# VikParuchuri/surya

Hardware: AMD Instinct MI355X
Metric: text-lines/sec recognised (whole node) (higher is better)
Workload: dtype bf16; 1 GPU; RecognitionPredictor device loop, 256 ragged 64x{128..512} crops/GPU, batch 256, max_tokens=48, REC-FULL synthetic weights (conditioned recipe, seed 0), tiles resident in HBM; parallelism=1 GPU, weights=conditioned

## Files before the change

### surya_amd/csrc/attn_mfma.h

```cpp
#pragma once
#include "common.h"
#include "kernels.h"

namespace sa {

typedef short s16x4 __attribute__((ext_vector_type(4)));

template <typename T, int D>
__global__ __launch_bounds__(128) void attn_mfma_kernel(const T* __restrict__ q, const T* __restrict__ k,
                                                        const T* __restrict__ v, T* __restrict__ out, AttnSegs sg,
                                                        long q_row, long q_head, long k_row, long k_head, long o_row, long o_head,
                                                        int group, int causal, float scale) {
    static_assert(D % 16 == 0 && D <= 128, "head dim");
    static_assert(sizeof(T) == 2, "16-bit storage types");
    constexpr int KC = 64;
    constexpr int PK = D + 8;
    constexpr int NKK = D / 16;
    constexpr int NDB = (D + 31) / 32;
    constexpr int CPR = D / 8;
    __shared__ __attribute__((aligned(16))) T ks[(KC + 1) * PK];
    __shared__ __attribute__((aligned(16))) T vs[(KC + 1) * PK];

    const int tile = blockIdx.x, head = blockIdx.y, kvh = head / group;
    const int seg = sg.tile_seg[tile], q0 = sg.tile_q0[tile], L = sg.seg_len[seg];
    const int tid = threadIdx.x, lane = tid & 63, wave = tid >> 6;
    const int ql = lane & 31, h = lane >> 5;
    const int qi = q0 + wave * 32 + ql;

    u32x4 qf[NKK];
    {
        const T* qp = q + sg.q_off[seg] + (long)min(qi, L - 1) * q_row + (long)head * q_head + h * 8;
#pragma unroll
        for (int kk = 0; kk < NKK; ++kk) qf[kk] = *reinterpret_cast<const u32x4*>(qp + kk * 16);
    }
    f32x16 oacc[NDB];
#pragma unroll
    for (int db = 0; db < NDB; ++db)
#pragma unroll
        for (int r = 0; r < 16; ++r) oacc[db][r] = 0.f;
    float mrun = -INFINITY, lrun = 0.f;
    const float sl2 = scale * 1.44269504088896340736f;

    const int kend = causal ? min(L, q0 + 64) : L;
    const T* kbase = k + sg.k_off[seg] + (long)kvh * k_head;
    const T* vbase = v + sg.v_off[seg] + (long)kvh * k_head;
    const int tr_off = ((lane & 15) >> 2) * PK + ((lane >> 4) & 1) * 16 + (lane & 3) * 4 + h * 4 * PK;

    constexpr int NST = KC * CPR / 128;
    static_assert(KC * CPR % 128 == 0, "staging split");
    u32x4 kreg[NST], vreg[NST];
    auto fetch = [&](int kc) {
        const int nk = min(KC, kend - kc);
#pragma unroll
        for (int it = 0; it < NST; ++it) {
            const int c = tid + it * 128, r = min(c / CPR, nk - 1), cc = c % CPR;
            kreg[it] = *reinterpret_cast<const u32x4*>(kbase + (long)(kc + r) * k_row + cc * 8);
            vreg[it] = *reinterpret_cast<const u32x4*>(vbase + (long)(kc + r) * k_row + cc * 8);
        }
    };
    if (kend > 0) fetch(0);
    for (int kc = 0; kc < kend; kc += KC) {
        const int nk = min(KC, kend - kc);
#pragma unroll
        for (int it = 0; it < NST; ++it) {
            const int c = tid + it * 128, r = c / CPR, cc = c % CPR;
            const bool in = r < nk;
            const u32x4 z = {0u, 0u, 0u, 0u};
            *reinterpret_cast<u32x4*>(ks + r * PK + cc * 8) = in ? kreg[it] : z;
            *reinterpret_cast<u32x4*>(vs + r * PK + cc * 8) = in ? vreg[it] : z;
        }
        __syncthreads();
        if (kc + KC < kend) fetch(kc + KC);

        f32x16 sacc[2];
#pragma unroll
        for (int kb = 0; kb < 2; ++kb) {
#pragma unroll
            for (int r = 0; r < 16; ++r) sacc[kb][r] = 0.f;
            const T* kp = ks + (kb * 32 + ql) * PK + h * 8;
#pragma unroll
            for (int kk = 0; kk < NKK; ++kk) {
                const u32x4 kf = *reinterpret_cast<const u32x4*>(kp + kk * 16);
                sacc[kb] = H16<T>::mfma(kf, qf[kk], sacc[kb]);
            }
        }
        float bm = -INFINITY;
#pragma unroll
        for (int kb = 0; kb < 2; ++kb)
#pragma unroll
            for (int g = 0; g < 4; ++g)
#pragma unroll
                for (int r = 0; r < 4; ++r) {
                    const int j = kb * 32 + g * 8 + h * 4 + r;
                    const bool ok = (j < nk) && (!causal || (kc + j) <= qi);
                    const float sv = ok ? sacc[kb][4 * g + r] : -INFINITY;
                    sacc[kb][4 * g + r] = sv;
                    bm = fmaxf(bm, sv);
                }
        bm = fmaxf(bm, __shfl_xor(bm, 32, 64));
        const float mnew = fmaxf(mrun, bm);
        const float alpha = exp2f((mrun - mnew) * sl2);
        mrun = mnew;
        float psum = 0.f;
#pragma unroll
        for (int kb = 0; kb < 2; ++kb)
#pragma unroll
            for (int r = 0; r < 16; ++r) {
                const float pv = exp2f((sacc[kb][r] - mnew) * sl2);
                sacc[kb][r] = pv;
                psum += pv;
            }
        lrun = lrun * alpha + psum;
#pragma unroll
        for (int db = 0; db < NDB; ++db)
#pragma unroll
            for (int r = 0; r < 16; ++r) oacc[db][r] *= alpha;

#pragma unroll
        for (int t = 0; t < 4; ++t) {
            const int kb = t >> 1, o8 = (t & 1) * 8;
            u32x4 pf;
            pf[0] = H16<T>::pk(sacc[kb][o8 + 0], sacc[kb][o8 + 1]);
            pf[1] = H16<T>::pk(sacc[kb][o8 + 2], sacc[kb][o8 + 3]);
            pf[2] = H16<T>::pk(sacc[kb][o8 + 4], sacc[kb][o8 + 5]);
            pf[3] = H16<T>::pk(sacc[kb][o8 + 6], sacc[kb][o8 + 7]);
#pragma unroll
            for (int db = 0; db < NDB; ++db) {
                const T* vp = vs + t * 16 * PK + db * 32 + tr_off;
                const s16x4 lo = __builtin_amdgcn_ds_read_tr16_b64_v4i16((__attribute__((address_space(3))) s16x4*)(vp));
                const s16x4 hi = __builtin_amdgcn_ds_read_tr16_b64_v4i16((__attribute__((address_space(3))) s16x4*)(vp + 8 * PK));
                typedef short s16x8 __attribute__((ext_vector_type(8)));
                const s16x8 vf = __builtin_shufflevector(lo, hi, 0, 1, 2, 3, 4, 5, 6, 7);
                oacc[db] = H16<T>::mfma(vf, pf, oacc[db]);
            }
        }
        __syncthreads();
    }

    const float ltot = lrun + __shfl_xor(lrun, 32, 64);
    if (qi < L) {
        const float inv = 1.0f / ltot;
        T* op = out + sg.o_off[seg] + (long)qi * o_row + (long)head * o_head;
#pragma unroll
        for (int db = 0; db < NDB; ++db)
#pragma unroll
            for (int g = 0; g < 4; ++g) {
                const int d0 = db * 32 + g * 8 + h * 4;
                if (d0 < D) store4(op + d0, oacc[db][4 * g] * inv, oacc[db][4 * g + 1] * inv, oacc[db][4 * g + 2] * inv,
                                   oacc[db][4 * g + 3] * inv);
            }
    }
}

template <typename T>
int launch_attn(int D, const T* q, const T* k, const T* v, T* o, const AttnSegs& sg, int n_tiles, int heads, long q_row, long q_head,
                long k_row, long k_head, long o_row, long o_head, int group, int causal, float scale, hipStream_t s) {
    if (n_tiles <= 0) return SA_OK;
    auto go = [&](auto kern, int threads) {
        hipLaunchKernelGGL(kern, dim3(n_tiles, heads), dim3(threads), 0, s, q, k, v, o, sg, q_row, q_head, k_row, k_head, o_row, o_head, group,
                           causal, scale);
        return (int)hipGetLastError();
    };
    if constexpr (sizeof(T) == 2) {
        if (D == 32) return go(attn_mfma_kernel<T, 32>, 128);
        if (D == 64) return go(attn_mfma_kernel<T, 64>, 128);
        if (D == 80) return go(attn_mfma_kernel<T, 80>, 128);
        if (D == 128) return go(attn_mfma_kernel<T, 128>, 128);
    } else {
        static_assert(std::is_same<T, float>::value, "the VALU kernel is the fp32 reference-mode path only");
        if (D == 32) return go(attn_valu_kernel<T, 32>, 256);
        if (D == 64) return go(attn_valu_kernel<T, 64>, 256);
        if (D == 80) return go(attn_valu_kernel<T, 80>, 256);
        if (D == 128) return go(attn_valu_kernel<T, 128>, 256);
    }
    return SA_ERR_UNSUPPORTED;
}

}
```

### surya_amd/csrc/common.h

```cpp
#pragma once
#include <hip/hip_runtime.h>
#include <cstdlib>
#include <stdint.h>
#include <stdio.h>
#include <type_traits>

#include "../../include/surya_amd.h"

namespace sa {

typedef unsigned short bf16_t;
typedef __attribute__((ext_vector_type(4))) float f32x4;
typedef __attribute__((ext_vector_type(16))) float f32x16;
typedef __attribute__((ext_vector_type(8))) __bf16 bf16x8;
typedef unsigned int u32x4 __attribute__((ext_vector_type(4)));


#define SA_HIP(expr)                                                                                   \
    do {                                                                                               \
        hipError_t _e = (expr);                                                                        \
        if (_e != hipSuccess) {                                                                        \
            fprintf(stderr, "[surya_amd] %s:%d %s -> %s\n", __FILE__, __LINE__, #expr, hipGetErrorString(_e)); \
            return (int)_e;                                                                            \
        }                                                                                              \
// ... 214 lines not shown
__device__ __forceinline__ float hardswish_f(float x) {
    float t;
    asm("v_fma_f32 %0, %1, %2, 0.5 clamp" : "=v"(t) : "v"(x), "s"(1.0f / 6.0f));
    return x * t;
}
typedef float f32x2_hs __attribute__((ext_vector_type(2)));
__device__ __forceinline__ f32x2_hs hardswish_pk(f32x2_hs x) {
    f32x2_hs t;
    const f32x2_hs c = {1.0f / 6.0f, 1.0f / 6.0f};
    asm("v_pk_fma_f32 %0, %1, %2, 0.5 op_sel_hi:[1,0,0] clamp" : "=v"(t) : "v"(x), "s"(c));
    return x * t;
}

struct Tuning {
    int graph = 0;
    int split_target = 256;
    int split_min_kt = 4;
    int split_max = 8;
    int bigtile = 3;
    int bigtile_any = 0;
    int big_m_split = -1;
    int big_m_gateup = -1;
    int mx_big_m_split = -1;
    int mx_big_m_gateup = -1;
    int gateup_ring = 2;
    int dring = 1;
    int dring_min_kt = 0;
    int conv_persist = 3;
    int dwconv_pipe = 2;
    int conv_lean = 1;
    int bigtile_ratio_pct = 0;
    int bigtile_min_k = 0;
    int glds = 2;
    int dattn = 4;
    int rnorm = 2;
    int ghead = 2;
    int fuse_embed = 1;
    int kvprefetch = 0;
    int lmhead = 1;
    int dattn_db = 0;
    int lay_ln = 1;
    int det_head_blk = 1;
    int det_fuse = 1023;
    int det_up4 = 1;
    int fmb_chunk = 64;
    int persist = 1;
    int ocrerr_cls_only = 1;
};
inline Tuning& tuning() { static Tuning t; return t; }
inline int& tuning_epoch() { static int e = 0; return e; }

inline void poison_arena(void* p, size_t bytes) {
    static const bool on = [] { const char* e = getenv("SURYA_AMD_POISON"); return e && e[0] == '1'; }();
    if (on) { (void)hipMemset(p, 0xFF, bytes); (void)hipDeviceSynchronize(); }
}

struct AttrOnce {
    size_t granted[64] = {};
    template <typename F> void ensure(F kern, size_t lds) {
        int dev = 0;
        (void)hipGetDevice(&dev);
        size_t& g = granted[dev & 63];
        if (lds > g || g == 0) {
            (void)hipFuncSetAttribute(reinterpret_cast<const void*>(kern), hipFuncAttributeMaxDynamicSharedMemorySize, (int)lds);
            g = lds > g ? lds : g;
            if (g == 0) g = 1;
        }
    }
};

constexpr int SA_ALT_NONE = 0x7fffffff;
__device__ __forceinline__ bool alt_after(float v, int c, float pv, int pc) { return (v < pv) | ((v == pv) & (c > pc)); }
__device__ __forceinline__ bool alt_before(float v, int c, float bv, int bc) { return (v > bv) | ((v == bv) & (c < bc)); }
__device__ __forceinline__ float2 alt_next(const float2* cand, int n, float pv, int pc) {
    float cb = -INFINITY;
    int ci = SA_ALT_NONE;
    for (int k = 0; k < n; ++k) {
        const float v = cand[k].x;
        const int cc = __float_as_int(cand[k].y);
// ... 12 lines not shown
```

### surya_amd/csrc/decode_attn.h

```cpp
#pragma once
#include "gemm.h"

namespace sa {

#ifdef SA_DA_TIMING
__device__ unsigned long long sa_da_stamps[16];
#define SA_DA_STAMP(i) if (blockIdx.x == 64 && blockIdx.y == 0 && threadIdx.x == 0) sa_da_stamps[i] = wall_clock64();
#else
#define SA_DA_STAMP(i)
#endif

template <typename T, int D, int MAXG>
__global__ __launch_bounds__(256) void decode_attn_mfma_kernel(const float* __restrict__ qkv_part, int S, const T* __restrict__ qkv_bias,
                                                               T* __restrict__ out, T* __restrict__ kc, T* __restrict__ vc,
                                                               const int* __restrict__ active_slots, const int* __restrict__ row_len,
                                                               const float2* __restrict__ rope_cs, int nq, int nkv, int Tmax,
                                                               float scale) {
    constexpr int V16 = Ty<T>::V16;
    constexpr int CPRk = D / V16;
    constexpr int ROWB = D * (int)sizeof(T);
    constexpr int KT = (ROWB >= 512) ? 64 : 128;
    constexpr int XM = CPRk >= 16 ? 15 : CPRk - 1;
    constexpr int NCH = KT * CPRk / 256;
    static_assert(KT * CPRk % 256 == 0 && NCH >= 1 && D % 32 == 0 && MAXG <= 32, "geometry");
// ... 407 lines not shown
    }
    __syncthreads();
    SA_DA_STAMP(6)
    if (tid < G * (D / 4)) {
        const int oh = tid / (D / 4), od = (tid % (D / 4)) * 4;
        float mx = -INFINITY;
#pragma unroll
        for (int w = 0; w < 4; ++w) mx = fmaxf(mx, comb[(w * MAXG + oh) * CW + D]);
        float num[4] = {0.f, 0.f, 0.f, 0.f}, den = 0.f;
#pragma unroll
        for (int w = 0; w < 4; ++w) {
            const float* rec = comb + (w * MAXG + oh) * CW;
            const float e = (rec[D] == -INFINITY) ? 0.f : __expf(rec[D] - mx);
            const float4 o4 = *reinterpret_cast<const float4*>(rec + od);
            num[0] += e * o4.x; num[1] += e * o4.y; num[2] += e * o4.z; num[3] += e * o4.w;
            den += e * rec[D + 1];
        }
        const float inv = 1.0f / den;
        const long o_off = (long)a * nq * D + (long)(kvh * G + oh) * D + od;
        store4(out + o_off, num[0] * inv, num[1] * inv, num[2] * inv, num[3] * inv);
        if (out8) {
            const float q[4] = {Ty<T>::rnd(num[0] * inv), Ty<T>::rnd(num[1] * inv), Ty<T>::rnd(num[2] * inv), Ty<T>::rnd(num[3] * inv)};
            int e8;
            const uint32_t pk = mx_quant4_oct(q, e8);
            *reinterpret_cast<uint32_t*>(out8 + o_off) = pk;
            const int col = (kvh * G + oh) * D + od;
            if ((tid & 7) == 0) sout[((long)(col >> 7) * srows + a) * 4 + ((col >> 5) & 3)] = (uint8_t)e8;
        }
    }
    SA_DA_STAMP(7)
    SA_DA_STAMP(8)
}

template <int D, int MAXG, bool DB = false, typename T = bf16_t>
__global__ __launch_bounds__(256) void decode_attn_flash2_kernel(const float* __restrict__ qkv_part, int S, const T* __restrict__ qkv_bias,
                                                                 T* __restrict__ out, T* __restrict__ kc, T* __restrict__ vc,
                                                                 const int* __restrict__ active_slots, const int* __restrict__ row_len,
                                                                 const float2* __restrict__ rope_cs, int nq, int nkv, int Tmax,
                                                                 float scale, uint8_t* __restrict__ out8 = nullptr,
                                                                 uint8_t* __restrict__ sout = nullptr, int srows = 0) {
    static_assert(sizeof(T) == 2, "a 16-bit storage type");
    constexpr int CPR = D / 8;
    constexpr int ROWB = D * 2;
    constexpr int KT = 128;
    constexpr int RPI = 1024 / ROWB;
    constexpr int XM = CPR >= 16 ? 15 : CPR - 1;
    constexpr int NKK = D / 16, NDB = (D + 31) / 32;
    constexpr int CW = D + 4;
    constexpr int IPH = D / 8;
    static_assert(D % 32 == 0 && D <= 128 && MAXG <= 32 && 1024 % ROWB == 0, "geometry");
    static_assert((MAXG + 2) * IPH <= 256 && MAXG * CW * 4 <= 32 * ROWB, "one prologue pass; a wave's records fit its own K rows");
    extern __shared__ __attribute__((aligned(16))) unsigned char smem[];
    constexpr int NBUF = DB ? 2 : 1;
    constexpr int BUFB = 2 * KT * ROWB;
    unsigned char* Ks = smem;
    unsigned char* Vs = Ks + KT * ROWB;
    unsigned char* qT = smem + NBUF * BUFB;

    SA_DA_STAMP(0)
    const int G = nq / nkv;
    const int a = blockIdx.x, kvh = blockIdx.y;
    const int slot = active_slots[a];
    const int len = row_len[a];
    const int tid = threadIdx.x, lane = tid & 63, wave = tid >> 6;
    const int total = len + 1;
    const unsigned char* kb = reinterpret_cast<const unsigned char*>(kc + ((long)slot * nkv + kvh) * Tmax * D);
    const unsigned char* vb = reinterpret_cast<const unsigned char*>(vc + ((long)slot * nkv + kvh) * Tmax * D);
    typedef const __attribute__((address_space(1))) void* gptr_t;
    typedef __attribute__((address_space(3))) void* lptr_t;

    auto issue_tile = [&](int base, int buf) {
        const int rows = min(KT, (total - base + 15) & ~15);
        const int ngroups = (rows + RPI - 1) / RPI;
        unsigned char* Kd = Ks + buf * BUFB;
        unsigned char* Vd = Vs + buf * BUFB;
        for (int g = wave; g < ngroups; g += 4) {
            const int r = g * RPI + lane / CPR, pc = lane % CPR;
            const long j = min(base + r, max(len - 1, 0));
            if (base + r != len) {
                __builtin_amdgcn_global_load_lds((gptr_t)(kb + j * ROWB + ((pc ^ (r & XM)) << 4)), (lptr_t)(Kd + g * 1024), 16, 0, 0);
                __builtin_amdgcn_global_load_lds((gptr_t)(vb + j * ROWB + (pc << 4)), (lptr_t)(Vd + g * 1024), 16, 0, 0);
            }
        }
    };
    issue_tile(0, 0);
    SA_DA_STAMP(1)

    const int qkv_dim = (nq + 2 * nkv) * D;
    const int Mrows = gridDim.x;
    constexpr int half = D / 2;
    const int n_items = (G + 2) * IPH;
    const int item = min(tid, n_items - 1);
    const bool on = tid < n_items;
    const int hh = item / IPH, i0 = (item % IPH) * 4;
    const int col = (hh < G ? (kvh * G + hh) * D : (hh == G ? (nq + kvh) * D : (nq + nkv + kvh) * D)) + i0;
    const float* prow = qkv_part + (long)a * qkv_dim + col;
    const long sstride = (long)Mrows * qkv_dim;
    f32x4 plo[8], phi[8];
    const int SL = S <= 2 ? 2 : (S <= 4 ? 4 : 8);
    if (SL == 2) {
#pragma unroll
        for (int s = 0; s < 2; ++s) {
            plo[s] = *reinterpret_cast<const f32x4*>(prow + min(s, S - 1) * sstride);
            phi[s] = *reinterpret_cast<const f32x4*>(prow + min(s, S - 1) * sstride + half);
        }
#pragma unroll
        for (int s = 2; s < 8; ++s) { plo[s] = f32x4{0.f, 0.f, 0.f, 0.f}; phi[s] = plo[s]; }
    } else if (SL == 4) {
#pragma unroll
        for (int s = 0; s < 4; ++s) {
            plo[s] = *reinterpret_cast<const f32x4*>(prow + min(s, S - 1) * sstride);
            phi[s] = *reinterpret_cast<const f32x4*>(prow + min(s, S - 1) * sstride + half);
        }
#pragma unroll
        for (int s = 4; s < 8; ++s) { plo[s] = f32x4{0.f, 0.f, 0.f, 0.f}; phi[s] = plo[s]; }
    } else {
#pragma unroll
        for (int s = 0; s < 8; ++s) {
            plo[s] = *reinterpret_cast<const f32x4*>(prow + min(s, S - 1) * sstride);
            phi[s] = *reinterpret_cast<const f32x4*>(prow + min(s, S - 1) * sstride + half);
        }
    }
    float blo[4], bhi[4];
    load4(qkv_bias + col, blo);
    load4(qkv_bias + col + half, bhi);
    const float4 csA = *reinterpret_cast<const float4*>(rope_cs + (long)len * half + i0);
    const float4 csB = *reinterpret_cast<const float4*>(rope_cs + (long)len * half + i0 + 2);
    for (int i = tid; i < (32 - G) * CPR; i += 256)
        *reinterpret_cast<u32x4*>(qT + G * ROWB + i * 16) = u32x4{0u, 0u, 0u, 0u};
    SA_DA_STAMP(2)
    float xlo[4], xhi[4];
#pragma unroll
    for (int e = 0; e < 4; ++e) {
        float vl = blo[e], vh = bhi[e];
#pragma unroll
        for (int s = 0; s < 8; ++s) {
            const bool use = s < S;
            vl += use ? plo[s][e] : 0.f;
            vh += use ? phi[s][e] : 0.f;
        }
        xlo[e] = Ty<T>::rnd(vl); xhi[e] = Ty<T>::rnd(vh);
    }
    const float csn[4] = {csA.x, csA.z, csB.x, csB.z}, snn[4] = {csA.y, csA.w, csB.y, csB.w};
    float ylo[4], yhi[4];
#pragma unroll
    for (int e = 0; e < 4; ++e) {
        const float r1 = Ty<T>::rnd(__fmaf_rn(xlo[e], csn[e], -__fmul_rn(xhi[e], snn[e])));
        const float r2 = Ty<T>::rnd(__fmaf_rn(xhi[e], csn[e], __fmul_rn(xlo[e], snn[e])));
        ylo[e] = hh <= G ? r1 : xlo[e];
        yhi[e] = hh <= G ? r2 : xhi[e];
    }
    const int new_tile = len / KT, new_row = len % KT;
    auto lds_put4 = [&](unsigned char* rowp, int swz, int e0, const float (&v)[4], float mul) {
        const int c = e0 / 8, w = e0 % 8;
        store4(reinterpret_cast<T*>(rowp + ((c ^ swz) << 4)) + w, v[0] * mul, v[1] * mul, v[2] * mul, v[3] * mul);
    };
    auto put_new_rows = [&](int buf) {
        if (on && hh == G) {
            lds_put4(Ks + buf * BUFB + new_row * ROWB, new_row & XM, i0, ylo, 1.f);
            lds_put4(Ks + buf * BUFB + new_row * ROWB, new_row & XM, i0 + half, yhi, 1.f);
        } else if (on && hh == G + 1) {
            lds_put4(Vs + buf * BUFB + new_row * ROWB, 0, i0, ylo, 1.f);
            lds_put4(Vs + buf * BUFB + new_row * ROWB, 0, i0 + half, yhi, 1.f);
        }
    };
    if (on && hh < G) {
        lds_put4(qT + hh * ROWB, hh & XM, i0, ylo, scale);
        lds_put4(qT + hh * ROWB, hh & XM, i0 + half, yhi, scale);
    }
    if (new_tile == 0) put_new_rows(0);
    SA_DA_STAMP(3)
    asm volatile("s_waitcnt vmcnt(0)" ::: "memory");
    __syncthreads();
    if (on && hh >= G) {
        T* dst = (hh == G ? kc : vc) + (((long)slot * nkv + kvh) * Tmax + len) * D;
// ... 152 lines not shown
static inline size_t decode_attn_mfma_lds() {
    constexpr int ROWB = D * (int)sizeof(T);
    constexpr int KT = (ROWB >= 512) ? 64 : 128;
    return (size_t)2 * KT * ROWB + 32 * ROWB + (size_t)MAXG * KT * 4 + (size_t)(MAXG + 2) * D * 4 + 3 * MAXG * 4 + 64;
}

template <typename T>
struct DecodeAttnArgs {
    const float* qkv_part; int S;
    const T* qkv_bias;
    T* out;
    T *kcache, *vcache;
    const int *active_slots, *row_len;
    const float2* rope_cs;
    int rows, nq, nkv, d, max_kv_len;
    float scale;
    int ctx_bound = 0;
    uint8_t *out8 = nullptr, *sout = nullptr; int srows = 0;
};
template <typename T>
int launch_decode_attn(const DecodeAttnArgs<T>& a, hipStream_t s);
template <> int launch_decode_attn<fp16_t>(const DecodeAttnArgs<fp16_t>& a, hipStream_t s);
int decode_attn_f16_d128(const DecodeAttnArgs<fp16_t>& a, hipStream_t s);

template <auto KERN, typename T, typename... X>
static int decode_attn_as(const DecodeAttnArgs<T>& a, size_t lds, hipStream_t s, X... extra) {
    static AttrOnce attr;
    attr.ensure(KERN, lds);
    hipLaunchKernelGGL(KERN, dim3(a.rows, a.nkv), dim3(256), lds, s, a.qkv_part, a.S, a.qkv_bias, a.out, a.kcache, a.vcache, a.active_slots,
                       a.row_len, a.rope_cs, a.nq, a.nkv, a.max_kv_len, a.scale, extra...);
    return (int)hipGetLastError();
}

}
```

### surya_amd/csrc/layout_model.hip

```cpp
#include <algorithm>
#include <cstring>
#include <map>
#include <memory>
#include <set>
#include <vector>

#include "../../include/surya_amd.h"
#include "gemm.h"
#include "kernels.h"
#include "decode_attn.h"
#include "layout_kernels.h"
#include "layout_prep.h"

namespace sa {

struct LayoutBase {
    virtual ~LayoutBase() {}
    virtual int encode(const float* pixels, int B, hipStream_t s) = 0;
    virtual int decode_step(const int32_t* boxes, int B, int pos, float* cls, float* box, hipStream_t s) = 0;
    virtual int encoder_states(void* out, int B, hipStream_t s) = 0;
    virtual int select(const int32_t* src, int n) = 0;
    virtual int prefill(const int32_t* boxes, int B, int Tn, float* cls, float* box, hipStream_t s) = 0;
    virtual int set_feedback(const surya_layout_feedback* fb, int B, hipStream_t s) = 0;
    virtual int decode_steps(const int32_t* boxes, int B, int pos0, int n_steps, int ring, hipStream_t s) = 0;
// ... 700 lines not shown
        const float* hb = hc + ring_cls;
        const int* ht = reinterpret_cast<const int*>(hb + ring_box);
        const int tw = tokw();
        for (int k = 0; k < n_steps; ++k) {
            memcpy(cls + (size_t)k * B * c.label_count, hc + (size_t)k * mb * c.label_count, (size_t)B * c.label_count * sizeof(float));
            memcpy(box + (size_t)k * B * 6, hb + (size_t)k * mb * 6, (size_t)B * 6 * sizeof(float));
            memcpy(tok + (size_t)k * B * tw, ht + (size_t)k * mb * 10, (size_t)B * tw * sizeof(int));
        }
        return SA_OK;
    }
};

}

namespace sa {
int op_gemm_geglu(int dtype, const void* X, long ldx, const void* W, long ldw, void* C, long ldc, int M, int N, int K, hipStream_t s) {
    if (dtype == SA_DTYPE_F32) {
        GemmArgs<float, float> a{(const float*)X, ldx, (const float*)W, ldw, (float*)C, ldc, nullptr, nullptr, 0, M, N, K};
        return launch_gemm<float, float, EPI_GEGLU>(a, s);
    }
    if (dtype == SA_DTYPE_BF16) {
        GemmArgs<bf16_t, bf16_t> a{(const bf16_t*)X, ldx, (const bf16_t*)W, ldw, (bf16_t*)C, ldc, nullptr, nullptr, 0, M, N, K};
        return launch_gemm<bf16_t, bf16_t, EPI_GEGLU>(a, s);
    }
    if (dtype == SA_DTYPE_F16) {
        GemmArgs<fp16_t, fp16_t> a{(const fp16_t*)X, ldx, (const fp16_t*)W, ldw, (fp16_t*)C, ldc, nullptr, nullptr, 0, M, N, K};
        return launch_gemm<fp16_t, fp16_t, EPI_GEGLU>(a, s);
    }
    return SA_ERR_UNSUPPORTED;
}

template <int D>
static int decode_attn_flash_f16(const DecodeAttnArgs<fp16_t>& a, hipStream_t s) {
    const Tuning& t = tuning();
    if (t.dattn_db == 1 || (t.dattn_db == 0 && !t.graph && a.ctx_bound > 128 && a.rows * a.nkv <= 256))
        return decode_attn_as<decode_attn_flash2_kernel<D, 8, true, fp16_t>>(a, decode_attn_flash2_lds<D, 8, true>(), s, a.out8, a.sout, a.srows);
    return decode_attn_as<decode_attn_flash2_kernel<D, 8, false, fp16_t>>(a, decode_attn_flash2_lds<D, 8, false>(), s, a.out8, a.sout, a.srows);
}
template <>
int launch_decode_attn<fp16_t>(const DecodeAttnArgs<fp16_t>& a, hipStream_t s) {
    const int G = a.nq / a.nkv;
    if (a.out8 || G < 1 || G > 8 || a.nq % a.nkv) return SA_ERR_UNSUPPORTED;
    if (a.d == 64) return decode_attn_flash_f16<64>(a, s);
    if (a.d == 32) return decode_attn_flash_f16<32>(a, s);
    if (a.d == 128) return decode_attn_f16_d128(a, s);
    return SA_ERR_UNSUPPORTED;
}
}

using namespace sa;
struct surya_layout { std::unique_ptr<LayoutBase> impl; };

extern "C" {

int surya_layout_create(const surya_layout_config* cfg, const void* const* weights, int n_weights, surya_layout** out) {
    if (!cfg || !weights || !out) return SA_ERR_ARG;
    if (cfg->n_stages < 1 || cfg->n_stages > 8 || cfg->patch * cfg->patch * 3 > 64 || cfg->embed_dim % 64 || cfg->window != 8) return SA_ERR_UNSUPPORTED;
    if (cfg->img_h % cfg->patch || cfg->img_w % cfg->patch || cfg->dec_hidden % 64 || cfg->dec_inter % 64 || cfg->dec_heads % cfg->dec_kv_heads)
        return SA_ERR_SHAPE;
    if (cfg->max_batch <= 0 || cfg->max_boxes <= 0 || cfg->label_count <= 0) return SA_ERR_ARG;
    if (cfg->vocab <= cfg->bbox_size) return SA_ERR_SHAPE;
    if (cfg->family != SA_FAMILY_LAYOUT && cfg->family != SA_FAMILY_TABLE) return SA_ERR_ARG;
    if (cfg->family == SA_FAMILY_TABLE &&
        (cfg->box_embed <= 0 || cfg->box_embed >= cfg->dec_hidden || cfg->category_count <= 0 || cfg->merge_count <= 0)) return SA_ERR_ARG;
    for (int i = 0; i < n_weights; ++i)
        if (!weights[i]) return SA_ERR_ARG;
    auto* h = new surya_layout();
    int rc;
    if (cfg->dtype == SA_DTYPE_F32) {
        auto m = std::make_unique<LayoutModel<float>>();
// ... 267 lines not shown
```

### surya_amd/csrc/rec_model.hip

```cpp
#include "rec_engine.h"
#include "rec_ops.h"
#include "rec_prep.h"

namespace sa {

template <int D, int MAXG>
static int decode_attn_flash(const DecodeAttnArgs<bf16_t>& a, hipStream_t s) {
    const Tuning& t = tuning();
    if (t.dattn == 3) return decode_attn_as<decode_attn_flash_kernel<D, MAXG>>(a, decode_attn_flash_lds<D, MAXG>(), s, a.out8, a.sout, a.srows);
    if (t.dattn_db == 1 || (t.dattn_db == 0 && !t.graph && a.ctx_bound > 128 && a.rows * a.nkv <= 256))
        return decode_attn_as<decode_attn_flash2_kernel<D, MAXG, true>>(a, decode_attn_flash2_lds<D, MAXG, true>(), s, a.out8, a.sout, a.srows);
    return decode_attn_as<decode_attn_flash2_kernel<D, MAXG, false>>(a, decode_attn_flash2_lds<D, MAXG, false>(), s, a.out8, a.sout, a.srows);
}
template <typename T>
int launch_decode_attn(const DecodeAttnArgs<T>& a, hipStream_t s) {
    const int G = a.nq / a.nkv, d = a.d;
    if constexpr (std::is_same<T, bf16_t>::value) {
        if (d == 128 && G <= 5) return decode_attn_flash<128, 5>(a, s);
        if (d == 128 && G <= 8) return decode_attn_flash<128, 8>(a, s);
        if (d == 64 && G <= 8) return decode_attn_flash<64, 8>(a, s);
        if (d == 32 && G <= 8) return decode_attn_flash<32, 8>(a, s);
    }
    if (a.out8) return SA_ERR_UNSUPPORTED;
    if (d == 128 && G <= 5) return decode_attn_as<decode_attn_mfma_kernel<T, 128, 5>>(a, decode_attn_mfma_lds<T, 128, 5>(), s);
    if (d == 128 && G <= 8) return decode_attn_as<decode_attn_mfma_kernel<T, 128, 8>>(a, decode_attn_mfma_lds<T, 128, 8>(), s);
    if (d == 64 && G <= 8) return decode_attn_as<decode_attn_mfma_kernel<T, 64, 8>>(a, decode_attn_mfma_lds<T, 64, 8>(), s);
    if (d == 32 && G <= 8) return decode_attn_as<decode_attn_mfma_kernel<T, 32, 8>>(a, decode_attn_mfma_lds<T, 32, 8>(), s);
    return SA_ERR_UNSUPPORTED;
}
template int launch_decode_attn<float>(const DecodeAttnArgs<float>&, hipStream_t);
template int launch_decode_attn<bf16_t>(const DecodeAttnArgs<bf16_t>&, hipStream_t);

static int check_cfg(const surya_rec_config* c) {
    if (!c) return SA_ERR_ARG;
    if (c->dtype != SA_DTYPE_F32 && c->dtype != SA_DTYPE_BF16 && c->dtype != SA_DTYPE_F16) return SA_ERR_UNSUPPORTED;
    if (c->enc_hidden % 64 || c->enc_inter_pad % 64 || c->patch_dim_pad % 64 || c->dec_hidden % 64 || c->dec_inter % 64 ||
        (c->dec_heads * c->dec_head_dim) % 64 || c->vocab % 4)
        return SA_ERR_SHAPE;
    if (c->enc_hidden % c->enc_heads || c->dec_heads % c->dec_kv_heads || c->dec_heads / c->dec_kv_heads > 8) return SA_ERR_SHAPE;
    if (c->merge != 2 || c->window_tokens <= 0 || c->enc_depth > 32) return SA_ERR_UNSUPPORTED;
    if (c->max_slots <= 0 || c->max_kv_len <= 0 || c->max_patches < 4 || c->max_prefill_tokens <= 0) return SA_ERR_ARG;
    return SA_OK;
}

}
// ... 465 lines not shown
        int rc = launch_gemm_mx_splitk(a, s);
        *splitk = a.splitk;
        return rc;
    }
    if (mode == 2) {
        if (!q_out || !sq_out) return SA_ERR_ARG;
        a.Q = q_out; a.ldq = N / 2; a.SQ = sq_out; a.sq_rows = M;
        return launch_gemm_mx<MX_EPI_SWIGLU>(a, s);
    }
    return SA_ERR_ARG;
}

int surya_rec_preprocess(const uint8_t* pages, const void* lines, int n_lines, uint8_t* mask_arena, float* mid_arena, float* tiles,
                         int patch_size, int merge_size, float pad_value, const float* mean, const float* std, int any_poly,
                         int max_stage1_width, int pixel_stride, void* stream) {
    if (!pages || !lines || !tiles || !mean || !std || n_lines < 0 || patch_size <= 0 || merge_size <= 0) return SA_ERR_ARG;
    if (pixel_stride != 3 && pixel_stride != 4) return SA_ERR_ARG;
    sa::prep::PrepArgs p;
    p.pages = pages; p.lines = reinterpret_cast<const sa::prep::LineDesc*>(lines); p.n_lines = n_lines;
    p.mask = mask_arena; p.mid = mid_arena; p.tiles = tiles; p.ps = patch_size; p.merge = merge_size; p.pad = pad_value;
    for (int i = 0; i < 3; ++i) { p.mean[i] = mean[i]; p.std[i] = std[i]; }
    p.max_mid_w = max_stage1_width;
    p.pix = pixel_stride;
    return sa::prep::prep_run(p, any_poly, max_stage1_width > 0, (hipStream_t)stream);
}

int surya_set_tuning(const char* key, int value) {
    if (!key) return SA_ERR_ARG;
    Tuning& t = tuning();
    struct { const char* k; int* v; } tab[] = {
        {"graph", &t.graph}, {"split_target", &t.split_target}, {"split_min_kt", &t.split_min_kt}, {"split_max", &t.split_max},
        {"bigtile", &t.bigtile}, {"bigtile_any", &t.bigtile_any}, {"conv_lean", &t.conv_lean}, {"conv_persist", &t.conv_persist}, {"dwconv_pipe", &t.dwconv_pipe}, {"bigtile_ratio_pct", &t.bigtile_ratio_pct}, {"gateup_ring", &t.gateup_ring}, {"dring", &t.dring}, {"dring_min_kt", &t.dring_min_kt}, {"big_m_split", &t.big_m_split}, {"big_m_gateup", &t.big_m_gateup}, {"mx_big_m_split", &t.mx_big_m_split}, {"mx_big_m_gateup", &t.mx_big_m_gateup}, {"glds", &t.glds}, {"bigtile_min_k", &t.bigtile_min_k}, {"dattn", &t.dattn}, {"rnorm", &t.rnorm},
        {"ghead", &t.ghead}, {"fuse_embed", &t.fuse_embed}, {"persist", &t.persist}, {"lmhead", &t.lmhead}, {"kvprefetch", &t.kvprefetch},
        {"dattn_db", &t.dattn_db}, {"lay_ln", &t.lay_ln}, {"det_head_blk", &t.det_head_blk}, {"det_fuse", &t.det_fuse}, {"det_up4", &t.det_up4}, {"fmb_chunk", &t.fmb_chunk}, {"ocrerr_cls_only", &t.ocrerr_cls_only}};
    for (auto& e : tab)
        if (!strcmp(e.k, key)) {
            if (*e.v != value) ++tuning_epoch();
            *e.v = value;
            return SA_OK;
        }
    return SA_ERR_ARG;
}

int surya_gemm_ring_status(int reset) {
    const int a = sa::ring_error(reset != 0), b = sa::rec_f16_ring_error(reset != 0);
    return a ? a : b;
}

int surya_prof_enable(int on) {
    GemmProfiler& pf = gemm_profiler();
    if (on) pf.start(); else pf.enabled = false;
    return SA_OK;
}

__global__ void prof_null_kernel() {}

int surya_prof_event_overhead(void* stream, double* ms) {
    if (!ms) return SA_ERR_ARG;
    hipStream_t s = (hipStream_t)stream;
    constexpr int N = 201;
    hipEvent_t ev[2 * N];
    for (auto& e : ev) SA_HIP(hipEventCreate(&e));
    for (int i = 0; i < 32; ++i) hipLaunchKernelGGL(prof_null_kernel, dim3(1), dim3(64), 0, s);
    for (int i = 0; i < N; ++i) {
        SA_HIP(hipEventRecord(ev[2 * i], s));
        hipLaunchKernelGGL(prof_null_kernel, dim3(1), dim3(64), 0, s);
        SA_HIP(hipEventRecord(ev[2 * i + 1], s));
// ... 100 lines not shown
```

### surya_amd/csrc/rec_model_f16.hip

```cpp
#include "rec_engine.h"
#include "rec_ops.h"

namespace sa {

template <int MAXG>
static int decode_attn_flash_f16_d128(const DecodeAttnArgs<fp16_t>& a, hipStream_t s) {
    const Tuning& t = tuning();
    if (t.dattn_db == 1 || (t.dattn_db == 0 && !t.graph && a.ctx_bound > 128 && a.rows * a.nkv <= 256))
        return decode_attn_as<decode_attn_flash2_kernel<128, MAXG, true, fp16_t>>(a, decode_attn_flash2_lds<128, MAXG, true>(), s, a.out8, a.sout, a.srows);
    return decode_attn_as<decode_attn_flash2_kernel<128, MAXG, false, fp16_t>>(a, decode_attn_flash2_lds<128, MAXG, false>(), s, a.out8, a.sout, a.srows);
}
int decode_attn_f16_d128(const DecodeAttnArgs<fp16_t>& a, hipStream_t s) {
    const int G = a.nq / a.nkv;
    if (a.d != 128 || a.out8 || G < 1 || a.nq % a.nkv) return SA_ERR_UNSUPPORTED;
    if (G <= 5) return decode_attn_flash_f16_d128<5>(a, s);
    if (G <= 8) return decode_attn_flash_f16_d128<8>(a, s);
    return SA_ERR_UNSUPPORTED;
}

size_t rec_f16_workspace_bytes(const surya_rec_config& cfg) { return RecModel<fp16_t>::layout(cfg, nullptr); }
int rec_f16_create(const surya_rec_config& cfg, const void* const* weights, int n, std::unique_ptr<RecBase>& out) {
    auto m = std::make_unique<RecModel<fp16_t>>();
    const int rc = m->init(cfg, weights, n);
    out = std::move(m);
    return rc;
}
int rec_f16_ring_error(bool reset) { return ring_error(reset); }

int op_lm_head_f16(const void* X, const void* W, const void* bias, int M, int N, int K, const TokenMask* tm, float4* amax, float2* alt, int* bn_used,
                   hipStream_t s, const ForcedCols* fc) {
    GemmArgs<fp16_t, float> a{(const fp16_t*)X, (long)K, (const fp16_t*)W, (long)K, nullptr, (long)N, (const fp16_t*)bias, nullptr, 0, M, N, K};
    a.amax = amax;
    int rc;
    if (fc) {
        a.forced = *fc;
        rc = launch_gemm<fp16_t, float, EPI_FORCED>(a, s);
    } else if (alt) {
        if (tm) a.tmask = *tm;
        a.alt = alt;
        rc = launch_gemm<fp16_t, float, EPI_TOPK>(a, s);
    } else if (tm) {
        a.tmask = *tm;
        rc = launch_gemm<fp16_t, float, EPI_ARGMAX_MASK>(a, s);
// ... 57 lines not shown
```

Measured before the change: 3132 lines/s.

## Remap attention blocks across XCDs and hoist decode QKV slab loads early

The prefill/encoder attention kernel can now launch on a 1D grid whose block index is remapped so consecutive tiles of the same head group spread across the 8 XCDs. By default this applies when k_row equals q_row, and the aim is better L2 locality and load balance for K/V reuse. Separately, the decode flash2 kernel gains an EARLY variant, enabled by making dattn default to 5, that issues the split-K QKV partial and bias loads before the KV tile fetch, so their latency overlaps the cache tile load. This costs more live registers early in the kernel and an extra template instantiation.

Result: faster. 3178 lines/s (median of 6 runs) (+1.5%).

```diff
diff --git a/surya_amd/csrc/attn_mfma.h b/surya_amd/csrc/attn_mfma.h
--- a/surya_amd/csrc/attn_mfma.h
+++ b/surya_amd/csrc/attn_mfma.h
@@ -1,4 +1,5 @@
 #pragma once
+#include "attn_order.h"
 #include "common.h"
 #include "kernels.h"
 
@@ -7,10 +8,92 @@
 typedef short s16x4 __attribute__((ext_vector_type(4)));
 
 template <typename T, int D>
+__device__ __forceinline__ void attn_chunk(const T* ks, const T* vs, const u32x4 (&qf)[D / 16], f32x16 (&oacc)[(D + 31) / 32], float& mrun,
+                                           float& lrun, int nk, int kc, int qi, int causal, float sl2, int ql, int h, int tr_off) {
+    constexpr int PK = D + 8, NKK = D / 16, NDB = (D + 31) / 32;
+    f32x16 sacc[2];
+#pragma unroll
+    for (int kb = 0; kb < 2; ++kb) {
+#pragma unroll
+        for (int r = 0; r < 16; ++r) sacc[kb][r] = 0.f;
+        const T* kp = ks + (kb * 32 + ql) * PK + h * 8;
+#pragma unroll
+        for (int kk = 0; kk < NKK; ++kk) {
+            const u32x4 kf = *reinterpret_cast<const u32x4*>(kp + kk * 16);
+            sacc[kb] = H16<T>::mfma(kf, qf[kk], sacc[kb]);
+        }
+    }
+    float bm = -INFINITY;
+#pragma unroll
+    for (int kb = 0; kb < 2; ++kb)
+#pragma unroll
+        for (int g = 0; g < 4; ++g)
+#pragma unroll
+            for (int r = 0; r < 4; ++r) {
+                const int j = kb * 32 + g * 8 + h * 4 + r;
+                const bool ok = (j < nk) && (!causal || (kc + j) <= qi);
+                const float sv = ok ? sacc[kb][4 * g + r] : -INFINITY;
+                sacc[kb][4 * g + r] = sv;
+                bm = fmaxf(bm, sv);
+            }
+    bm = fmaxf(bm, __shfl_xor(bm, 32, 64));
+    const float mnew = fmaxf(mrun, bm);
+    const float alpha = exp2f((mrun - mnew) * sl2);
+    mrun = mnew;
+    float psum = 0.f;
+#pragma unroll
+    for (int kb = 0; kb < 2; ++kb)
+#pragma unroll
+        for (int r = 0; r < 16; ++r) {
+            const float pv = exp2f((sacc[kb][r] - mnew) * sl2);
+            sacc[kb][r] = pv;
+            psum += pv;
+        }
+    lrun = lrun * alpha + psum;
+#pragma unroll
+    for (int db = 0; db < NDB; ++db)
+#pragma unroll
+        for (int r = 0; r < 16; ++r) oacc[db][r] *= alpha;
+
+#pragma unroll
+    for (int t = 0; t < 4; ++t) {
+        const int kb = t >> 1, o8 = (t & 1) * 8;
+        u32x4 pf;
+        pf[0] = H16<T>::pk(sacc[kb][o8 + 0], sacc[kb][o8 + 1]);
+        pf[1] = H16<T>::pk(sacc[kb][o8 + 2], sacc[kb][o8 + 3]);
+        pf[2] = H16<T>::pk(sacc[kb][o8 + 4], sacc[kb][o8 + 5]);
+        pf[3] = H16<T>::pk(sacc[kb][o8 + 6], sacc[kb][o8 + 7]);
+#pragma unroll
+        for (int db = 0; db < NDB; ++db) {
+            const T* vp = vs + t * 16 * PK + db * 32 + tr_off;
+            const s16x4 lo = __builtin_amdgcn_ds_read_tr16_b64_v4i16((__attribute__((address_space(3))) s16x4*)(vp));
+            const s16x4 hi = __builtin_amdgcn_ds_read_tr16_b64_v4i16((__attribute__((address_space(3))) s16x4*)(vp + 8 * PK));
+            typedef short s16x8 __attribute__((ext_vector_type(8)));
+            const s16x8 vf = __builtin_shufflevector(lo, hi, 0, 1, 2, 3, 4, 5, 6, 7);
+            oacc[db] = H16<T>::mfma(vf, pf, oacc[db]);
+        }
+    }
+}
+
+template <typename T, int D>
+__device__ __forceinline__ void attn_store(T* op, const f32x16 (&oacc)[(D + 31) / 32], float ltot, int h) {
+    constexpr int NDB = (D + 31) / 32;
+    const float inv = 1.0f / ltot;
+#pragma unroll
+    for (int db = 0; db < NDB; ++db)
+#pragma unroll
+        for (int g = 0; g < 4; ++g) {
+            const int d0 = db * 32 + g * 8 + h * 4;
+            if (d0 < D) store4(op + d0, oacc[db][4 * g] * inv, oacc[db][4 * g + 1] * inv, oacc[db][4 * g + 2] * inv,
+                               oacc[db][4 * g + 3] * inv);
+        }
+}
+
+template <typename T, int D>
 __global__ __launch_bounds__(128) void attn_mfma_kernel(const T* __restrict__ q, const T* __restrict__ k,
                                                         const T* __restrict__ v, T* __restrict__ out, AttnSegs sg,
                                                         long q_row, long q_head, long k_row, long k_head, long o_row, long o_head,
-                                                        int group, int causal, float scale) {
+                                                        int group, int causal, float scale, int n_tiles, int heads, int order) {
     static_assert(D % 16 == 0 && D <= 128, "head dim");
     static_assert(sizeof(T) == 2, "16-bit storage types");
     constexpr int KC = 64;
@@ -21,7 +104,9 @@
     __shared__ __attribute__((aligned(16))) T ks[(KC + 1) * PK];
     __shared__ __attribute__((aligned(16))) T vs[(KC + 1) * PK];
 
-    const int tile = blockIdx.x, head = blockIdx.y, kvh = head / group;
+    int tile = blockIdx.x, head = blockIdx.y;
+    if (order && !attn_order_map(blockIdx.x, n_tiles, heads, tile, head)) return;
+    const int kvh = head / group;
     const int seg = sg.tile_seg[tile], q0 = sg.tile_q0[tile], L = sg.seg_len[seg];
     const int tid = threadIdx.x, lane = tid & 63, wave = tid >> 6;
     const int ql = lane & 31, h = lane >> 5;
@@ -71,107 +156,42 @@
         }
         __syncthreads();
         if (kc + KC < kend) fetch(kc + KC);
-
-        f32x16 sacc[2];
-#pragma unroll
-        for (int kb = 0; kb < 2; ++kb) {
-#pragma unroll
-            for (int r = 0; r < 16; ++r) sacc[kb][r] = 0.f;
-            const T* kp = ks + (kb * 32 + ql) * PK + h * 8;
-#pragma unroll
-            for (int kk = 0; kk < NKK; ++kk) {
-                const u32x4 kf = *reinterpret_cast<const u32x4*>(kp + kk * 16);
-                sacc[kb] = H16<T>::mfma(kf, qf[kk], sacc[kb]);
-            }
-        }
-        float bm = -INFINITY;
-#pragma unroll
-        for (int kb = 0; kb < 2; ++kb)
-#pragma unroll
-            for (int g = 0; g < 4; ++g)
-#pragma unroll
-                for (int r = 0; r < 4; ++r) {
-                    const int j = kb * 32 + g * 8 + h * 4 + r;
-                    const bool ok = (j < nk) && (!causal || (kc + j) <= qi);
-                    const float sv = ok ? sacc[kb][4 * g + r] : -INFINITY;
-                    sacc[kb][4 * g + r] = sv;
-                    bm = fmaxf(bm, sv);
-                }
-        bm = fmaxf(bm, __shfl_xor(bm, 32, 64));
-        const float mnew = fmaxf(mrun, bm);
-        const float alpha = exp2f((mrun - mnew) * sl2);
-        mrun = mnew;
-        float psum = 0.f;
-#pragma unroll
-        for (int kb = 0; kb < 2; ++kb)
-#pragma unroll
-            for (int r = 0; r < 16; ++r) {
-                const float pv = exp2f((sacc[kb][r] - mnew) * sl2);
-                sacc[kb][r] = pv;
-                psum += pv;
-            }
-        lrun = lrun * alpha + psum;
-#pragma unroll
-        for (int db = 0; db < NDB; ++db)
-#pragma unroll
-            for (int r = 0; r < 16; ++r) oacc[db][r] *= alpha;
-
-#pragma unroll
-        for (int t = 0; t < 4; ++t) {
-            const int kb = t >> 1, o8 = (t & 1) * 8;
-            u32x4 pf;
-            pf[0] = H16<T>::pk(sacc[kb][o8 + 0], sacc[kb][o8 + 1]);
-            pf[1] = H16<T>::pk(sacc[kb][o8 + 2], sacc[kb][o8 + 3]);
-            pf[2] = H16<T>::pk(sacc[kb][o8 + 4], sacc[kb][o8 + 5]);
-            pf[3] = H16<T>::pk(sacc[kb][o8 + 6], sacc[kb][o8 + 7]);
-#pragma unroll
-            for (int db = 0; db < NDB; ++db) {
-                const T* vp = vs + t * 16 * PK + db * 32 + tr_off;
-                const s16x4 lo = __builtin_amdgcn_ds_read_tr16_b64_v4i16((__attribute__((address_space(3))) s16x4*)(vp));
-                const s16x4 hi = __builtin_amdgcn_ds_read_tr16_b64_v4i16((__attribute__((address_space(3))) s16x4*)(vp + 8 * PK));
-                typedef short s16x8 __attribute__((ext_vector_type(8)));
-                const s16x8 vf = __builtin_shufflevector(lo, hi, 0, 1, 2, 3, 4, 5, 6, 7);
-                oacc[db] = H16<T>::mfma(vf, pf, oacc[db]);
-            }
-        }
+        attn_chunk<T, D>(ks, vs, qf, oacc, mrun, lrun, nk, kc, qi, causal, sl2, ql, h, tr_off);
         __syncthreads();
     }
 
     const float ltot = lrun + __shfl_xor(lrun, 32, 64);
-    if (qi < L) {
-        const float inv = 1.0f / ltot;
-        T* op = out + sg.o_off[seg] + (long)qi * o_row + (long)head * o_head;
-#pragma unroll
-        for (int db = 0; db < NDB; ++db)
-#pragma unroll
-            for (int g = 0; g < 4; ++g) {
-                const int d0 = db * 32 + g * 8 + h * 4;
-                if (d0 < D) store4(op + d0, oacc[db][4 * g] * inv, oacc[db][4 * g + 1] * inv, oacc[db][4 * g + 2] * inv,
-                                   oacc[db][4 * g + 3] * inv);
-            }
-    }
+    if (qi < L) attn_store<T, D>(out + sg.o_off[seg] + (long)qi * o_row + (long)head * o_head, oacc, ltot, h);
 }
 
 template <typename T>
 int launch_attn(int D, const T* q, const T* k, const T* v, T* o, const AttnSegs& sg, int n_tiles, int heads, long q_row, long q_head,
                 long k_row, long k_head, long o_row, long o_head, int group, int causal, float scale, hipStream_t s) {
     if (n_tiles <= 0) return SA_OK;
-    auto go = [&](auto kern, int threads) {
-        hipLaunchKernelGGL(kern, dim3(n_tiles, heads), dim3(threads), 0, s, q, k, v, o, sg, q_row, q_head, k_row, k_head, o_row, o_head, group,
-                           causal, scale);
-        return (int)hipGetLastError();
-    };
     if constexpr (sizeof(T) == 2) {
-        if (D == 32) return go(attn_mfma_kernel<T, 32>, 128);
-        if (D == 64) return go(attn_mfma_kernel<T, 64>, 128);
-        if (D == 80) return go(attn_mfma_kernel<T, 80>, 128);
-        if (D == 128) return go(attn_mfma_kernel<T, 128>, 128);
+        const int knob = tuning().attn_order;
+        const int order = knob >= 2 || (knob == 1 && k_row == q_row);
+        auto go = [&](auto kern) {
+            const dim3 grid = order ? dim3((unsigned)attn_order_grid(n_tiles, heads, 1)) : dim3(n_tiles, heads);
+            hipLaunchKernelGGL(kern, grid, dim3(128), 0, s, q, k, v, o, sg, q_row, q_head, k_row, k_head, o_row, o_head, group, causal, scale,
+                               n_tiles, heads, order);
+            return (int)hipGetLastError();
+        };
+        if (D == 32) return go(attn_mfma_kernel<T, 32>);
+        if (D == 64) return go(attn_mfma_kernel<T, 64>);
+        if (D == 80) return go(attn_mfma_kernel<T, 80>);
+        if (D == 128) return go(attn_mfma_kernel<T, 128>);
     } else {
         static_assert(std::is_same<T, float>::value, "the VALU kernel is the fp32 reference-mode path only");
-        if (D == 32) return go(attn_valu_kernel<T, 32>, 256);
-        if (D == 64) return go(attn_valu_kernel<T, 64>, 256);
-        if (D == 80) return go(attn_valu_kernel<T, 80>, 256);
-        if (D == 128) return go(attn_valu_kernel<T, 128>, 256);
+        auto go = [&](auto kern) {
+            hipLaunchKernelGGL(kern, dim3(n_tiles, heads), dim3(256), 0, s, q, k, v, o, sg, q_row, q_head, k_row, k_head, o_row, o_head, group,
+                               causal, scale);
+            return (int)hipGetLastError();
+        };
+        if (D == 32) return go(attn_valu_kernel<T, 32>);
+        if (D == 64) return go(attn_valu_kernel<T, 64>);
+        if (D == 80) return go(attn_valu_kernel<T, 80>);
+        if (D == 128) return go(attn_valu_kernel<T, 128>);
     }
     return SA_ERR_UNSUPPORTED;
 }
diff --git a/surya_amd/csrc/attn_order.h b/surya_amd/csrc/attn_order.h
--- /dev/null
+++ b/surya_amd/csrc/attn_order.h
@@ -0,0 +1,25 @@
+#pragma once
+
+#if defined(__HIPCC__)
+#define SA_AO_HD __host__ __device__ inline
+#else
+#define SA_AO_HD inline
+#endif
+
+namespace sa {
+
+constexpr int ATTN_XCDS = 8;
+
+SA_AO_HD int attn_head_groups(int heads, int hpw) { return (heads + hpw - 1) / hpw; }
+SA_AO_HD long attn_order_grid(int n_tiles, int heads, int hpw) {
+    return (long)((n_tiles + ATTN_XCDS - 1) / ATTN_XCDS) * ATTN_XCDS * attn_head_groups(heads, hpw);
+}
+SA_AO_HD bool attn_order_map(long b, int n_tiles, int n_groups, int& tile, int& hg) {
+    const int x = (int)(b % ATTN_XCDS);
+    const long j = b / ATTN_XCDS;
+    hg = (int)(j % n_groups);
+    tile = (int)(j / n_groups) * ATTN_XCDS + x;
+    return tile < n_tiles;
+}
+
+}
diff --git a/surya_amd/csrc/common.h b/surya_amd/csrc/common.h
--- a/surya_amd/csrc/common.h
+++ b/surya_amd/csrc/common.h
@@ -270,7 +270,7 @@
     int bigtile_ratio_pct = 0;
     int bigtile_min_k = 0;
     int glds = 2;
-    int dattn = 4;
+    int dattn = 5;
     int rnorm = 2;
     int ghead = 2;
     int fuse_embed = 1;
@@ -283,6 +283,7 @@
     int det_up4 = 1;
     int fmb_chunk = 64;
     int persist = 1;
+    int attn_order = 1;
     int ocrerr_cls_only = 1;
 };
 inline Tuning& tuning() { static Tuning t; return t; }
diff --git a/surya_amd/csrc/decode_attn.h b/surya_amd/csrc/decode_attn.h
--- a/surya_amd/csrc/decode_attn.h
+++ b/surya_amd/csrc/decode_attn.h
@@ -463,7 +463,7 @@
     SA_DA_STAMP(8)
 }
 
-template <int D, int MAXG, bool DB = false, typename T = bf16_t>
+template <int D, int MAXG, bool DB = false, typename T = bf16_t, bool EARLY = false>
 __global__ __launch_bounds__(256) void decode_attn_flash2_kernel(const float* __restrict__ qkv_part, int S, const T* __restrict__ qkv_bias,
                                                                  T* __restrict__ out, T* __restrict__ kc, T* __restrict__ vc,
                                                                  const int* __restrict__ active_slots, const int* __restrict__ row_len,
@@ -491,9 +491,56 @@
     SA_DA_STAMP(0)
     const int G = nq / nkv;
     const int a = blockIdx.x, kvh = blockIdx.y;
+    const int tid = threadIdx.x, lane = tid & 63, wave = tid >> 6;
+    const int qkv_dim = (nq + 2 * nkv) * D;
+    const int Mrows = gridDim.x;
+    constexpr int half = D / 2;
+    const int n_items = (G + 2) * IPH;
+    const int item = min(tid, n_items - 1);
+    const bool on = tid < n_items;
+    const int hh = item / IPH, i0 = (item % IPH) * 4;
+    const int col = (hh < G ? (kvh * G + hh) * D : (hh == G ? (nq + kvh) * D : (nq + nkv + kvh) * D)) + i0;
+    const float* prow = qkv_part + (long)a * qkv_dim + col;
+    const long sstride = (long)Mrows * qkv_dim;
+    f32x4 plo[8], phi[8];
+    float blo[4], bhi[4];
+    const int SL = S <= 2 ? 2 : (S <= 4 ? 4 : 8);
+    auto slab = [&](int s, int off) { return *reinterpret_cast<const f32x4*>(prow + min(s, S - 1) * sstride + off); };
+    auto load_slabs = [&]() {
+        if (SL == 2) {
+#pragma unroll
+            for (int s = 0; s < 2; ++s) { plo[s] = slab(s, 0); phi[s] = slab(s, half); }
+#pragma unroll
+            for (int s = 2; s < 8; ++s) { plo[s] = f32x4{0.f, 0.f, 0.f, 0.f}; phi[s] = plo[s]; }
+        } else if (SL == 4) {
+#pragma unroll
+            for (int s = 0; s < 4; ++s) { plo[s] = slab(s, 0); phi[s] = slab(s, half); }
+#pragma unroll
+            for (int s = 4; s < 8; ++s) { plo[s] = f32x4{0.f, 0.f, 0.f, 0.f}; phi[s] = plo[s]; }
+        } else {
+#pragma unroll
+            for (int s = 0; s < 8; ++s) { plo[s] = slab(s, 0); phi[s] = slab(s, half); }
+        }
+        load4(qkv_bias + col, blo);
+        load4(qkv_bias + col + half, bhi);
+    };
+    auto load_slabs_early = [&]() {
+#pragma unroll
+        for (int s = 0; s < 2; ++s) { plo[s] = slab(s, 0); phi[s] = slab(s, half); }
+        if (SL > 2) {
+#pragma unroll
+            for (int s = 2; s < 4; ++s) { plo[s] = slab(s, 0); phi[s] = slab(s, half); }
+        }
+        if (SL > 4) {
+#pragma unroll
+            for (int s = 4; s < 8; ++s) { plo[s] = slab(s, 0); phi[s] = slab(s, half); }
+        }
+        load4(qkv_bias + col, blo);
+        load4(qkv_bias + col + half, bhi);
+    };
     const int slot = active_slots[a];
     const int len = row_len[a];
-    const int tid = threadIdx.x, lane = tid & 63, wave = tid >> 6;
+    if constexpr (EARLY) load_slabs_early();
     const int total = len + 1;
     const unsigned char* kb = reinterpret_cast<const unsigned char*>(kc + ((long)slot * nkv + kvh) * Tmax * D);
     const unsigned char* vb = reinterpret_cast<const unsigned char*>(vc + ((long)slot * nkv + kvh) * Tmax * D);
@@ -517,61 +564,39 @@
     issue_tile(0, 0);
     SA_DA_STAMP(1)
 
-    const int qkv_dim = (nq + 2 * nkv) * D;
-    const int Mrows = gridDim.x;
-    constexpr int half = D / 2;
-    const int n_items = (G + 2) * IPH;
-    const int item = min(tid, n_items - 1);
-    const bool on = tid < n_items;
-    const int hh = item / IPH, i0 = (item % IPH) * 4;
-    const int col = (hh < G ? (kvh * G + hh) * D : (hh == G ? (nq + kvh) * D : (nq + nkv + kvh) * D)) + i0;
-    const float* prow = qkv_part + (long)a * qkv_dim + col;
-    const long sstride = (long)Mrows * qkv_dim;
-    f32x4 plo[8], phi[8];
-    const int SL = S <= 2 ? 2 : (S <= 4 ? 4 : 8);
-    if (SL == 2) {
-#pragma unroll
-        for (int s = 0; s < 2; ++s) {
-            plo[s] = *reinterpret_cast<const f32x4*>(prow + min(s, S - 1) * sstride);
-            phi[s] = *reinterpret_cast<const f32x4*>(prow + min(s, S - 1) * sstride + half);
-        }
-#pragma unroll
-        for (int s = 2; s < 8; ++s) { plo[s] = f32x4{0.f, 0.f, 0.f, 0.f}; phi[s] = plo[s]; }
-    } else if (SL == 4) {
-#pragma unroll
-        for (int s = 0; s < 4; ++s) {
-            plo[s] = *reinterpret_cast<const f32x4*>(prow + min(s, S - 1) * sstride);
-            phi[s] = *reinterpret_cast<const f32x4*>(prow + min(s, S - 1) * sstride + half);
-        }
-#pragma unroll
-        for (int s = 4; s < 8; ++s) { plo[s] = f32x4{0.f, 0.f, 0.f, 0.f}; phi[s] = plo[s]; }
-    } else {
-#pragma unroll
-        for (int s = 0; s < 8; ++s) {
-            plo[s] = *reinterpret_cast<const f32x4*>(prow + min(s, S - 1) * sstride);
-            phi[s] = *reinterpret_cast<const f32x4*>(prow + min(s, S - 1) * sstride + half);
-        }
-    }
-    float blo[4], bhi[4];
-    load4(qkv_bias + col, blo);
-    load4(qkv_bias + col + half, bhi);
+    if constexpr (!EARLY) load_slabs();
     const float4 csA = *reinterpret_cast<const float4*>(rope_cs + (long)len * half + i0);
     const float4 csB = *reinterpret_cast<const float4*>(rope_cs + (long)len * half + i0 + 2);
     for (int i = tid; i < (32 - G) * CPR; i += 256)
         *reinterpret_cast<u32x4*>(qT + G * ROWB + i * 16) = u32x4{0u, 0u, 0u, 0u};
     SA_DA_STAMP(2)
     float xlo[4], xhi[4];
-#pragma unroll
-    for (int e = 0; e < 4; ++e) {
-        float vl = blo[e], vh = bhi[e];
-#pragma unroll
-        for (int s = 0; s < 8; ++s) {
-            const bool use = s < S;
-            vl += use ? plo[s][e] : 0.f;
-            vh += use ? phi[s][e] : 0.f;
-        }
-        xlo[e] = Ty<T>::rnd(vl); xhi[e] = Ty<T>::rnd(vh);
-    }
+    float vl[4], vh[4];
+#pragma unroll
+    for (int e = 0; e < 4; ++e) { vl[e] = blo[e]; vh[e] = bhi[e]; }
+    auto add_slabs = [&](int s0, int s1) {
+#pragma unroll
+        for (int e = 0; e < 4; ++e)
+#pragma unroll
+            for (int s = s0; s < s1; ++s) {
+                const bool use = s < S;
+                vl[e] += use ? plo[s][e] : 0.f;
+                vh[e] += use ? phi[s][e] : 0.f;
+            }
+    };
+    if constexpr (EARLY) {
+        add_slabs(0, 2);
+        if (SL > 2) add_slabs(2, 4);
+        if (SL > 4) add_slabs(4, 8);
+        if (S < 8) {
+#pragma unroll
+            for (int e = 0; e < 4; ++e) { vl[e] += 0.f; vh[e] += 0.f; }
+        }
+    } else {
+        add_slabs(0, 8);
+    }
+#pragma unroll
+    for (int e = 0; e < 4; ++e) { xlo[e] = Ty<T>::rnd(vl[e]); xhi[e] = Ty<T>::rnd(vh[e]); }
     const float csn[4] = {csA.x, csA.z, csB.x, csB.z}, snn[4] = {csA.y, csA.w, csB.y, csB.w};
     float ylo[4], yhi[4];
 #pragma unroll
@@ -790,4 +815,15 @@
     return (int)hipGetLastError();
 }
 
+template <int D, int MAXG, typename T>
+static int decode_attn_flash2_launch(const DecodeAttnArgs<T>& a, hipStream_t s) {
+    const Tuning& t = tuning();
+    const bool db = t.dattn_db == 1 || (t.dattn_db == 0 && !t.graph && a.ctx_bound > 128 && a.rows * a.nkv <= 256);
+    const bool early = t.dattn >= 5;
+    if (db && early) return decode_attn_as<decode_attn_flash2_kernel<D, MAXG, true, T, true>>(a, decode_attn_flash2_lds<D, MAXG, true>(), s, a.out8, a.sout, a.srows);
+    if (db) return decode_attn_as<decode_attn_flash2_kernel<D, MAXG, true, T, false>>(a, decode_attn_flash2_lds<D, MAXG, true>(), s, a.out8, a.sout, a.srows);
+    if (early) return decode_attn_as<decode_attn_flash2_kernel<D, MAXG, false, T, true>>(a, decode_attn_flash2_lds<D, MAXG, false>(), s, a.out8, a.sout, a.srows);
+    return decode_attn_as<decode_attn_flash2_kernel<D, MAXG, false, T, false>>(a, decode_attn_flash2_lds<D, MAXG, false>(), s, a.out8, a.sout, a.srows);
 }
+
+}
diff --git a/surya_amd/csrc/layout_model.hip b/surya_amd/csrc/layout_model.hip
--- a/surya_amd/csrc/layout_model.hip
+++ b/surya_amd/csrc/layout_model.hip
@@ -756,10 +756,7 @@
 
 template <int D>
 static int decode_attn_flash_f16(const DecodeAttnArgs<fp16_t>& a, hipStream_t s) {
-    const Tuning& t = tuning();
-    if (t.dattn_db == 1 || (t.dattn_db == 0 && !t.graph && a.ctx_bound > 128 && a.rows * a.nkv <= 256))
-        return decode_attn_as<decode_attn_flash2_kernel<D, 8, true, fp16_t>>(a, decode_attn_flash2_lds<D, 8, true>(), s, a.out8, a.sout, a.srows);
-    return decode_attn_as<decode_attn_flash2_kernel<D, 8, false, fp16_t>>(a, decode_attn_flash2_lds<D, 8, false>(), s, a.out8, a.sout, a.srows);
+    return decode_attn_flash2_launch<D, 8, fp16_t>(a, s);
 }
 template <>
 int launch_decode_attn<fp16_t>(const DecodeAttnArgs<fp16_t>& a, hipStream_t s) {
diff --git a/surya_amd/csrc/rec_model.hip b/surya_amd/csrc/rec_model.hip
--- a/surya_amd/csrc/rec_model.hip
+++ b/surya_amd/csrc/rec_model.hip
@@ -8,9 +8,7 @@
 static int decode_attn_flash(const DecodeAttnArgs<bf16_t>& a, hipStream_t s) {
     const Tuning& t = tuning();
     if (t.dattn == 3) return decode_attn_as<decode_attn_flash_kernel<D, MAXG>>(a, decode_attn_flash_lds<D, MAXG>(), s, a.out8, a.sout, a.srows);
-    if (t.dattn_db == 1 || (t.dattn_db == 0 && !t.graph && a.ctx_bound > 128 && a.rows * a.nkv <= 256))
-        return decode_attn_as<decode_attn_flash2_kernel<D, MAXG, true>>(a, decode_attn_flash2_lds<D, MAXG, true>(), s, a.out8, a.sout, a.srows);
-    return decode_attn_as<decode_attn_flash2_kernel<D, MAXG, false>>(a, decode_attn_flash2_lds<D, MAXG, false>(), s, a.out8, a.sout, a.srows);
+    return decode_attn_flash2_launch<D, MAXG, bf16_t>(a, s);
 }
 template <typename T>
 int launch_decode_attn(const DecodeAttnArgs<T>& a, hipStream_t s) {
@@ -542,7 +540,7 @@
         {"graph", &t.graph}, {"split_target", &t.split_target}, {"split_min_kt", &t.split_min_kt}, {"split_max", &t.split_max},
         {"bigtile", &t.bigtile}, {"bigtile_any", &t.bigtile_any}, {"conv_lean", &t.conv_lean}, {"conv_persist", &t.conv_persist}, {"dwconv_pipe", &t.dwconv_pipe}, {"bigtile_ratio_pct", &t.bigtile_ratio_pct}, {"gateup_ring", &t.gateup_ring}, {"dring", &t.dring}, {"dring_min_kt", &t.dring_min_kt}, {"big_m_split", &t.big_m_split}, {"big_m_gateup", &t.big_m_gateup}, {"mx_big_m_split", &t.mx_big_m_split}, {"mx_big_m_gateup", &t.mx_big_m_gateup}, {"glds", &t.glds}, {"bigtile_min_k", &t.bigtile_min_k}, {"dattn", &t.dattn}, {"rnorm", &t.rnorm},
         {"ghead", &t.ghead}, {"fuse_embed", &t.fuse_embed}, {"persist", &t.persist}, {"lmhead", &t.lmhead}, {"kvprefetch", &t.kvprefetch},
-        {"dattn_db", &t.dattn_db}, {"lay_ln", &t.lay_ln}, {"det_head_blk", &t.det_head_blk}, {"det_fuse", &t.det_fuse}, {"det_up4", &t.det_up4}, {"fmb_chunk", &t.fmb_chunk}, {"ocrerr_cls_only", &t.ocrerr_cls_only}};
+        {"dattn_db", &t.dattn_db}, {"attn_order", &t.attn_order}, {"lay_ln", &t.lay_ln}, {"det_head_blk", &t.det_head_blk}, {"det_fuse", &t.det_fuse}, {"det_up4", &t.det_up4}, {"fmb_chunk", &t.fmb_chunk}, {"ocrerr_cls_only", &t.ocrerr_cls_only}};
     for (auto& e : tab)
         if (!strcmp(e.k, key)) {
             if (*e.v != value) ++tuning_epoch();
diff --git a/surya_amd/csrc/rec_model_f16.hip b/surya_amd/csrc/rec_model_f16.hip
--- a/surya_amd/csrc/rec_model_f16.hip
+++ b/surya_amd/csrc/rec_model_f16.hip
@@ -5,10 +5,7 @@
 
 template <int MAXG>
 static int decode_attn_flash_f16_d128(const DecodeAttnArgs<fp16_t>& a, hipStream_t s) {
-    const Tuning& t = tuning();
-    if (t.dattn_db == 1 || (t.dattn_db == 0 && !t.graph && a.ctx_bound > 128 && a.rows * a.nkv <= 256))
-        return decode_attn_as<decode_attn_flash2_kernel<128, MAXG, true, fp16_t>>(a, decode_attn_flash2_lds<128, MAXG, true>(), s, a.out8, a.sout, a.srows);
-    return decode_attn_as<decode_attn_flash2_kernel<128, MAXG, false, fp16_t>>(a, decode_attn_flash2_lds<128, MAXG, false>(), s, a.out8, a.sout, a.srows);
+    return decode_attn_flash2_launch<128, MAXG, fp16_t>(a, s);
 }
 int decode_attn_f16_d128(const DecodeAttnArgs<fp16_t>& a, hipStream_t s) {
     const int G = a.nq / a.nkv;
```
